# fnysalehi/Surface-Irradiance-Estimation-from-Neural-Radiance-Fields

Hardware: AMD Instinct MI355X
Metric: Mrays/s @1080p NeRF inference (Lego snapshot); PSNR vs reference (higher is better)
Workload: dtype f16; 1 GPU; Lego-shaped synthetic scene (HashGrid L8 F4 T2^19 b=2.0, density MLP 32-64-16, rgb MLP 32-64-64-16, aabb_scale 1), 1920x1080 pinhole camera fov_x 0.6911 rad, 8 orbit azimuths, 1 spp, render_mode Shade, min_transmittance 0.01; frames_in_flight=2

## Files before the change

__graft_entry__.py:

```python
import importlib
import os
import sys

ROOT = os.path.dirname(os.path.abspath(__file__))
PKG = "surface-irradiance-estimation-from-neural-radiance-fields_amd"
if ROOT not in sys.path:
    sys.path.insert(0, ROOT)


def _pkg(sub):
    return importlib.import_module(PKG + "." + sub)


def build():
    lib = _pkg("build").build()
    _pkg("build").build(legacy=True)
    _pkg("build").build_pyngp()
    _pkg("build").build_main()
    sys.path.insert(0, os.path.join(ROOT, "oracle"))
    import oracle as orc

    orc.build()
    native = _pkg("native")
    L = native.load_library()
    missing = [s for s in native.EXPORTS if not hasattr(L, s)]
    if missing:
        raise RuntimeError(f"libngp_hip.so lacks symbols: {missing}")
    print(f"built {lib}; {L.ngp_version().decode()}")


def smoke():
    import numpy as np

    sys.path.insert(0, os.path.join(ROOT, "oracle"))
    import oracle as orc

    native, synthetic, scene = _pkg("native"), _pkg("synthetic"), _pkg("scene")
    sc = synthetic.make_scene(aabb_scale=1, seed=7, log2_hashmap_size=15)
    ctx = native.Context(0)
    ctx.set_model(sc)
    w, h = 96, 54
    mat = scene.orbit_camera(45.0)
    focal = scene.focal_from_fov_x(w, 0.6911)
    img, depth = ctx.render(native.make_camera(mat, w, h, focal), native.make_opts(), want_depth=True)
    st = ctx.render_stats()
    o = orc.Oracle()
    bf, _ = o.density_grid_to_bitfield(np.asarray(sc["density_grid"], np.float16).astype(np.float32), sc["max_cascade"])
    sc["density_grid_bitfield"] = bf
    m = o.make_model(sc)
# ... 30 lines not shown
```

surface-irradiance-estimation-from-neural-radiance-fields_amd/build.py:

```python
import os
import subprocess
import sys

HERE = os.path.dirname(os.path.abspath(__file__))
CSRC = os.path.join(HERE, "csrc")
LIB = os.path.join(HERE, "libngp_hip.so")
SOURCES = ["nerf_kernels.hip", "wide_kernels.hip", "mesh_kernels.hip", "train_kernels.hip", "mc_kernels.hip", "ngp_api.cpp", "ngp_model.cpp", "ngp_snapshot.cpp", "ngp_dataset.cpp", "ngp_render.cpp", "ngp_mesh.cpp", "ngp_train.cpp", "ngp_multi.cpp", "ngp_mc.cpp"]
FLAGS = ["--offload-arch=gfx950", "-O3", "-std=c++17", "-fPIC", "-shared", "-ffp-contract=off", "-fno-slp-vectorize", "-fvisibility=hidden", "-Wall", "-Wno-unused-function"]


def hipcc():
    for c in (os.environ.get("HIPCC"), "/opt/rocm/bin/hipcc", "hipcc"):
        if c and (os.path.isabs(c) and os.path.exists(c) or not os.path.isabs(c)):
            return c
    raise RuntimeError("hipcc not found")


LIB_LEGACY = os.path.join(HERE, "libngp_hip_legacy.so")


def needs_build(lib=LIB):
    if not os.path.exists(lib):
        return True
    t = os.path.getmtime(lib)
    for f in os.listdir(CSRC):
        if os.path.getmtime(os.path.join(CSRC, f)) > t:
            return True
    inc = os.path.join(HERE, "..", "include", "ngp_hip.h")
    return os.path.getmtime(inc) > t


def build(force=False, verbose=False, legacy=False):
    lib = LIB_LEGACY if legacy else LIB
    if not force and not needs_build(lib):
        return lib
    srcs = [os.path.join(CSRC, s) for s in SOURCES if os.path.exists(os.path.join(CSRC, s))]
    tmp = "%s.%d.tmp" % (lib, os.getpid())
    cmd = [hipcc()] + FLAGS + (["-DNGP_TCNN_LEGACY_ENCODE"] if legacy else []) + os.environ.get("NGP_BUILD_DEFINES", "").split() + ["-o", tmp] + srcs + ["-lz"]
    if verbose:
        print(" ".join(cmd))
    r = subprocess.run(cmd, capture_output=True, text=True)
    if r.returncode != 0:
        sys.stderr.write(r.stdout + r.stderr)
        if os.path.exists(tmp):
            os.remove(tmp)
        raise RuntimeError("hipcc failed")
    os.replace(tmp, lib)
    return lib


def pyngp_path():
    import sysconfig

    return os.path.join(HERE, "pyngp" + sysconfig.get_config_var("EXT_SUFFIX"))


def build_pyngp(force=False, verbose=False):
    import pybind11
    import sysconfig

    out = pyngp_path()
    srcs = [os.path.join(CSRC, "pyngp.cpp"), os.path.join(CSRC, "testbed_shim.h"), os.path.join(HERE, "..", "include", "ngp_hip.h")]
    if not force and os.path.exists(out) and all(os.path.getmtime(out) >= os.path.getmtime(s) for s in srcs):
        return out
    build()
    cmd = ["g++", "-O2", "-std=c++17", "-shared", "-fPIC", "-fvisibility=hidden", "-I", sysconfig.get_paths()["include"], "-I", pybind11.get_include(),
           srcs[0], "-o", out + ".%d.tmp" % os.getpid(), "-L", HERE, "-lngp_hip", "-Wl,-rpath,$ORIGIN"]
    if verbose:
        print(" ".join(cmd))
    r = subprocess.run(cmd, capture_output=True, text=True)
    if r.returncode != 0:
# ... 41 lines not shown
```

surface-irradiance-estimation-from-neural-radiance-fields_amd/csrc/nerf_device.h:

```cpp
#pragma once

#include "ngp_kernels.h"

namespace ngp {

typedef _Float16 half_t;
typedef _Float16 half8 __attribute__((ext_vector_type(8)));
typedef float floatx4 __attribute__((ext_vector_type(4)));

struct f3 {
	float x, y, z;
};

#define NGP_DEV __device__ __forceinline__

NGP_DEV f3 mk3(float x, float y, float z) { return f3{x, y, z}; }
NGP_DEV f3 add3(f3 a, f3 b) { return mk3(a.x + b.x, a.y + b.y, a.z + b.z); }
NGP_DEV f3 sub3(f3 a, f3 b) { return mk3(a.x - b.x, a.y - b.y, a.z - b.z); }
NGP_DEV f3 mul3(f3 a, f3 b) { return mk3(a.x * b.x, a.y * b.y, a.z * b.z); }
NGP_DEV f3 div3(f3 a, f3 b) { return mk3(a.x / b.x, a.y / b.y, a.z / b.z); }
NGP_DEV f3 scale3(f3 a, float s) { return mk3(a.x * s, a.y * s, a.z * s); }
NGP_DEV f3 adds3(f3 a, float s) { return mk3(a.x + s, a.y + s, a.z + s); }
NGP_DEV float dot3(f3 a, f3 b) { return (a.x * b.x + a.y * b.y) + a.z * b.z; }
NGP_DEV f3 normalize3(f3 a) {
	float len = __builtin_sqrtf(dot3(a, a));
	return mk3(a.x / len, a.y / len, a.z / len);
}
NGP_DEV f3 m3_mulv(const float* m, f3 v) {
	f3 r = mk3(m[0] * v.x, m[1] * v.x, m[2] * v.x);
	r = add3(r, mk3(m[3] * v.y, m[4] * v.y, m[5] * v.y));
	r = add3(r, mk3(m[6] * v.z, m[7] * v.z, m[8] * v.z));
	return r;
}

NGP_DEV uint32_t laine_karras_permutation(uint32_t x, uint32_t seed) {
// ... 603 lines not shown
}
NGP_DEV float product_hi(float w, uint32_t packed) {
	float p;
	asm("v_fma_mix_f32 %0, %1, %2, 0 op_sel:[0,1,0] op_sel_hi:[0,1,0]" : "=v"(p) : "v"(w), "v"(packed));
	return p;
}
NGP_DEV void accumulate_corner(uint2 v, float w, FeatureAcc& r) {
#ifndef NGP_TCNN_LEGACY_ENCODE
	const half2_t wh = {(half_t)w, (half_t)w};
	const uint32_t wv = __builtin_bit_cast(uint32_t, wh);
	uint32_t a01 = __builtin_bit_cast(uint32_t, r.f01), a23 = __builtin_bit_cast(uint32_t, r.f23);
	asm("v_pk_fma_f16 %0, %1, %2, %0" : "+v"(a01) : "v"(wv), "v"(v.x));
	asm("v_pk_fma_f16 %0, %1, %2, %0" : "+v"(a23) : "v"(wv), "v"(v.y));
	r.f01 = __builtin_bit_cast(half2_t, a01);
	r.f23 = __builtin_bit_cast(half2_t, a23);
#else
	half2_t a, b;
	a[0] = (half_t)product_lo(w, v.x);
	a[1] = (half_t)product_hi(w, v.x);
	b[0] = (half_t)product_lo(w, v.y);
	b[1] = (half_t)product_hi(w, v.y);
	r.f01 = r.f01 + a;
	r.f23 = r.f23 + b;
#endif
}
NGP_DEV void store_features(const FeatureAcc& lo, const FeatureAcc& hi, half8& out) {
	out[0] = lo.f01[0]; out[1] = lo.f01[1]; out[2] = lo.f23[0]; out[3] = lo.f23[1];
	out[4] = hi.f01[0]; out[5] = hi.f01[1]; out[6] = hi.f23[0]; out[7] = hi.f23[1];
}

struct EncodeInFlight {
	uint2 v[16];
	float wx[2], wy[2], wz[2];
};
NGP_DEV void encode_issue(GridRsrc grid, GridRsrc xgrid, const LevelInfo* lv, int h, float x, float y, float z, EncodeInFlight& e) {
	const LevelInfo& L0 = lv[h];
	const LevelInfo& L1 = lv[h + 4];
	const CellPos p0 = level_cell(L0, x, y, z), p1 = level_cell(L1, x, y, z);
	CornerSet c0, c1;
	if (__all((int)level_in_xor_range(L0, p0) & (int)level_in_xor_range(L1, p1))) {
		level_corners_xor(L0, p0, c0);
		level_corners_xor(L1, p1, c1);
#pragma unroll
		for (int c = 0; c < 8; ++c) e.v[c] = gather8(xgrid, c0.index[c]);
#pragma unroll
		for (int c = 0; c < 8; ++c) e.v[8 + c] = gather8(xgrid, c1.index[c]);
#if defined(NGP_EXPERIMENT_EXTRA_GATHERS)
#pragma unroll
		for (int c = 0; c < NGP_EXPERIMENT_EXTRA_GATHERS; ++c) {
			const uint2 d = gather8(xgrid, c & 1 ? c1.index[c & 7] : c0.index[c & 7]);
			asm volatile("" ::"v"(d.x), "v"(d.y));
		}
#endif
	} else {
		level_corners(L0, p0, c0);
		level_corners(L1, p1, c1);
#pragma unroll
		for (int c = 0; c < 8; ++c) e.v[c] = gather8(grid, c0.index[c]);
#pragma unroll
		for (int c = 0; c < 8; ++c) e.v[8 + c] = gather8(grid, c1.index[c]);
	}
	e.wx[0] = p0.wx; e.wy[0] = p0.wy; e.wz[0] = p0.wz;
	e.wx[1] = p1.wx; e.wy[1] = p1.wy; e.wz[1] = p1.wz;
}
NGP_DEV half8 encode_finish(const EncodeInFlight& e) {
	FeatureAcc acc[2] = {{{0, 0}, {0, 0}}, {{0, 0}, {0, 0}}};
#pragma unroll
	for (int l = 0; l < 2; ++l) {
		CellPos p;
		p.gx = p.gy = p.gz = 0;
		p.wx = e.wx[l]; p.wy = e.wy[l]; p.wz = e.wz[l];
		float w[8];
		corner_weights(p, w);
#pragma unroll
		for (int c = 0; c < 8; ++c) accumulate_corner(e.v[8 * l + c], w[c], acc[l]);
	}
	half8 out;
	store_features(acc[0], acc[1], out);
	return out;
}
NGP_DEV half8 encode_level_pair(GridRsrc grid, GridRsrc xgrid, const LevelInfo* lv, int h, float x, float y, float z) {
	EncodeInFlight e;
	encode_issue(grid, xgrid, lv, h, x, y, z, e);
	return encode_finish(e);
}

NGP_DEV void sh4_quad(int h, float dx01, float dy01, float dz01, float* out4) {
	float x = dx01 * 2.0f - 1.0f, y = dy01 * 2.0f - 1.0f, z = dz01 * 2.0f - 1.0f;
	float xy = x * y, xz = x * z, yz = y * z, x2 = x * x, y2 = y * y, z2 = z * z;
	float o[16];
	o[0] = 0.28209479177387814f;
	o[1] = -0.48860251190291987f * y;
	o[2] = 0.48860251190291987f * z;
	o[3] = -0.48860251190291987f * x;
	o[4] = 1.0925484305920792f * xy;
	o[5] = -1.0925484305920792f * yz;
	o[6] = 0.94617469575755997f * z2 - 0.31539156525251999f;
	o[7] = -1.0925484305920792f * xz;
	o[8] = 0.54627421529603959f * x2 - 0.54627421529603959f * y2;
	o[9] = 0.59004358992664352f * y * (-3.0f * x2 + y2);
	o[10] = 2.8906114426405538f * xy * z;
	o[11] = 0.45704579946446572f * y * (1.0f - 5.0f * z2);
	o[12] = 0.3731763325901154f * z * (5.0f * z2 - 3.0f);
	o[13] = 0.45704579946446572f * x * (1.0f - 5.0f * z2);
	o[14] = 1.4453057213202769f * z * (x2 - y2);
	o[15] = 0.59004358992664352f * x * (-x2 + 3.0f * y2);
#pragma unroll
	for (int j = 0; j < 4; ++j) {
		float a = h == 0 ? o[j] : o[4 + j];
		float b = h == 2 ? o[8 + j] : o[12 + j];
		out4[j] = h < 2 ? a : b;
	}
}
// ... 255 lines not shown
```

surface-irradiance-estimation-from-neural-radiance-fields_amd/csrc/nerf_kernels.hip:

```cpp
#include "render_common.h"
#include "pcg32.h"

namespace ngp {

constexpr int BLOCK = 256;

struct FusedGeneric {
	static constexpr bool probe = false, unit = false, outside = true, plain = false, normals = false;
	static constexpr int prof = 0, mips = (int)NERF_CASCADES, rgb_mid = 1;
};
struct FusedUnit : FusedGeneric { static constexpr bool unit = true; static constexpr int mips = 1; };
struct FusedUnitPlain : FusedUnit { static constexpr bool plain = true; };
struct FusedC5 : FusedGeneric { static constexpr bool outside = false; static constexpr int mips = 4; };
struct FusedC5Plain : FusedC5 { static constexpr bool plain = true; };
struct FusedMid0 : FusedGeneric { static constexpr int rgb_mid = 0; };
struct FusedMid2 : FusedGeneric { static constexpr int rgb_mid = 2; };
struct FusedLinRgb : FusedGeneric { static constexpr int rgb_mid = -1; };
struct FusedLin : FusedGeneric { static constexpr int rgb_mid = -2; };
struct FusedNormals : FusedGeneric { static constexpr bool normals = true; };
struct FusedProf : FusedGeneric { static constexpr int prof = 1; };
struct FusedUnitPlainProf : FusedUnitPlain { static constexpr int prof = 1; };
struct FusedUnitPlainProf2 : FusedUnitPlain { static constexpr int prof = 2; };
struct FusedProbe : FusedGeneric { static constexpr bool probe = true; };

template <class V>
NGP_DEV void fused_body(const ModelParams& M, const CameraParams& C, const FrameParams& F, const ProbeParams& P) {
	constexpr bool PROBE = V::probe, UNIT = V::unit, OUTSIDE = V::outside, PLAIN = V::plain, NORMALS = V::normals;
	constexpr int PROF = V::prof, MIPS = V::mips, RGB_MID = V::rgb_mid;
	const uint32_t max_cascade = UNIT ? 0u : M.max_cascade;
	const float cone_angle = UNIT ? 0.0f : M.cone_angle;
	const Stepping stepping = make_stepping(cone_angle);
	__shared__ uint4 s_w[n_frags_for(RGB_MID) * 64];
	__shared__ LevelInfo s_lv[N_LEVELS];
	__shared__ uint32_t s_coarse[MIPS * COARSE_WORDS_PER_MIP];
	__shared__ uint32_t s_coarse16[(UNIT ? 1 : (int)NERF_CASCADES) * 16];
	__shared__ uint2 s_sh[BLOCK * 4];
	constexpr int SLOTS = 64;
	__shared__ float4 s_samp[BLOCK / 64 * SLOTS];
	__shared__ uint2 s_res[BLOCK / 64 * SLOTS];
	__shared__ float4 s_nrm[NORMALS ? BLOCK / 64 * SLOTS : 1];
	__shared__ uint32_t s_xstate, s_xcount, s_active;
	constexpr uint32_t XRAYS = 16;
	__shared__ float s_xray[XRAYS * 16];
	if (threadIdx.x == 0) {
		s_xstate = 0u;
		s_xcount = 0u;
		s_active = BLOCK / 64;
	}
	unsigned long long t_entry = 0, rt_entry = 0;
	if (PROF) { t_entry = stamp(); rt_entry = realtime(); }
	for (int i = threadIdx.x; i < n_frags_for(RGB_MID) * 64; i += BLOCK) s_w[i] = M.wfrags[i];
	if (threadIdx.x < N_LEVELS) s_lv[threadIdx.x] = M.levels[threadIdx.x];
	for (uint32_t i = threadIdx.x; i < (max_cascade + 1 < (uint32_t)MIPS ? max_cascade + 1 : (uint32_t)MIPS) * COARSE_WORDS_PER_MIP; i += BLOCK) s_coarse[i] = M.coarse[i];
	if (threadIdx.x < (UNIT ? 1 : (int)NERF_CASCADES) * 16) s_coarse16[threadIdx.x] = M.coarse[NERF_CASCADES * COARSE_WORDS_PER_MIP + threadIdx.x];
	__syncthreads();

	const int lane = threadIdx.x & 63;
	const int c = lane & 15;
	if (lane == 0 && (threadIdx.x >> 6) == 0) atomicMax(&F.results[4], ~realtime());
	const GridRsrc t_grid = make_grid_rsrc(M.grid, M.grid_bytes), t_xgrid = make_grid_rsrc(M.xgrid, M.xgrid_bytes);
	const float* cam_last = (!PLAIN && C.moving) ? C.m1 : C.m;
	const f3 cam_fwd = mk3(cam_last[6], cam_last[7], cam_last[8]);
	const f3 bg_linear = (PROBE || !F.direct) ? mk3(0.f, 0.f, 0.f)
	                     : F.color_space == 1 ? mk3(F.background[0], F.background[1], F.background[2])
	                                          : mk3(srgb_to_linear(F.background[0]), srgb_to_linear(F.background[1]), srgb_to_linear(F.background[2]));
	const float4 empty_pixel = (!PROBE && F.direct) ? tonemap_pixel(F, bg_linear, 0.f, 0.f, 0.f, 0.f) : make_float4(0.f, 0.f, 0.f, 0.f);
	const f3 cam_pos = mk3(cam_last[9], cam_last[10], cam_last[11]);
	const f3 amin = mk3(M.aabb_min[0], M.aabb_min[1], M.aabb_min[2]);
	const f3 adiag = mk3(M.aabb_diag[0], M.aabb_diag[1], M.aabb_diag[2]);

	RayState ray;
	ray.alive = false;
	ray.o = ray.d = mk3(0.f, 0.f, 0.f);
	ray.t = 0.f;
	ray.idx = 0;
	ray.out = 0;
	f3 idir = mk3(0.f, 0.f, 0.f);
	Accum acc = {0.f, 0.f, 0.f, 0.f, 0.f, 0.f};
	uint32_t step = 1;
	uint32_t skip_i = 1;
	float t_max = 0.f;
	bool counted = false;
	uint32_t n_pend = 0, sl_lo = 0, sl_hi = 0;
	bool left_box = false;
	uint32_t n_slots = 0;
	const int wave_base = threadIdx.x & ~63;
	OccBlock occ_cache;
	occ_cache.key = 0xffffffffu;
	occ_cache.bits = make_uint2(0u, 0u);
	bool finished = false;
	bool idle = false;
	const uint32_t my_wave = threadIdx.x >> 6;

	bool exhausted = false;
	uint32_t qsel = (uint32_t)__builtin_amdgcn_s_getreg(20 | (0 << 6) | (3 << 11)) & 7u;
	int stall = 0;
	uint32_t n_alive_init = 0, n_hit = 0, n_samples = 0;
	unsigned long long p_skip[3] = {0, 0, 0};
	unsigned long long pt[4] = {0, 0, 0, 0}, p_iters = 0, p_passes = 0, p_rounds = 0, p_lane_steps = 0, t0 = 0, t1 = 0;

	unsigned long long rt_start = 0;
	if (PROF && F.prof) {
		rt_start = realtime();
		if (lane == 0) atomicMax(&F.prof[8], ~rt_start);
	}
	int tr_slot = -1;
	uint32_t tr_it = 0, tr_info0 = 0, tr_info1 = 0, tr_march = 0;
	uint32_t tr_net[5] = {0, 0, 0, 0, 0};
	unsigned long long tr_t[5] = {0, 0, 0, 0, 0};
	auto trace_emit = [&](int upto) {
		if (!PROF || tr_slot < 0) return;
		if (tr_it < F.trace_cap_iters && lane == 0) {
			uint32_t* r = F.trace + 16 + F.trace_cap_waves * 16u + ((size_t)tr_slot * F.trace_cap_iters + tr_it) * 16u;
			r[0] = (uint32_t)tr_t[0];
			for (int k = 1; k < 5; ++k) r[k] = (uint32_t)(tr_t[k <= upto ? k : upto] - tr_t[0]);
			r[5] = tr_info0;
			r[6] = tr_info1;
			r[7] = tr_march;
			for (int k = 0; k < 5; ++k) r[8 + k] = upto >= 3 ? tr_net[k] : 0u;
		}
		++tr_it;
	};
	for (;;) {
		if (PROF) { t0 = stamp(); tr_t[0] = t0; tr_info0 = tr_info1 = tr_march = 0; for (int k = 0; k < 5; ++k) tr_net[k] = 0; }
		unsigned long long dead_mask = __ballot(!ray.alive);
		int n_dead = __popcll(dead_mask);
		if ((exhausted || n_dead >= F.tune[0]) && __any(finished)) {
			bool hit = false;
			if (finished) {
				hit = shade_ray<PROBE, PLAIN, NORMALS>(F, P, bg_linear, ray.out, acc, step - 1u, ray.d);
				finished = false;
			}
			n_hit += (uint32_t)__popcll(__ballot(hit));
			if (PROF) tr_info1 |= 4u << 24;
		}
		if (!exhausted && n_dead >= (F.tune[0] > 16 ? F.tune[0] : 16)) {
			const uint32_t want = (uint32_t)n_dead >> 4, n_strips = F.n_local_tiles * 4u;
			uint32_t first = 0, limit = n_strips;
			if (!PROBE && F.xqueue) {
				for (int tries = 0; tries < 8; ++tries) {
					const uint32_t lo = (uint32_t)(((unsigned long long)n_strips * qsel) >> 3), hi = (uint32_t)(((unsigned long long)n_strips * (qsel + 1u)) >> 3);
					uint32_t off = 0;
					if (lane == 0) off = atomicAdd(F.xqueue + qsel, want);
					off = __builtin_amdgcn_readfirstlane(off);
					first = lo + off;
					limit = hi;
					if (off < hi - lo) break;
					first = limit = n_strips;
					qsel = (qsel + 1u) & 7u;
				}
			} else {
				if (lane == 0) first = atomicAdd(F.queue, want);
				first = __builtin_amdgcn_readfirstlane(first);
			}
			if (first >= limit) {
				exhausted = true;
			} else {
// ... 282 lines not shown
		const int hq = lane >> 4;
		auto sample_of = [&](int p, float& sx, float& sy, float& sz, Sh4& shq) {
			const float4 a = s_samp[wave_base + 16 * p + c];
			const uint32_t owner = s_res[wave_base + 16 * p + c].x;
			sx = a.x; sy = a.y; sz = a.z;
			union { uint2 u; half_t h[4]; } cv;
			cv.u = s_sh[(wave_base + (int)owner) * 4 + hq];
#pragma unroll
			for (int j = 0; j < 4; ++j) shq.v[j] = cv.h[j];
		};
		auto deliver = [&](int p, const MlpOut& mo) {
			union { half_t h[4]; uint2 u; } o;
			o.h[0] = mo.rgb[0]; o.h[1] = mo.rgb[1]; o.h[2] = mo.rgb[2]; o.h[3] = mo.sigma;
			if (lane < 16) s_res[wave_base + 16 * p + lane] = o.u;
		};
		int p = 0;
		if (NORMALS) {
			for (; p < n_pass; ++p) {
				float ax, ay, az;
				Sh4 sha;
				sample_of(p, ax, ay, az, sha);
				EncodeInFlight e;
				encode_issue(t_grid, t_xgrid, s_lv, hq, ax, ay, az, e);
				const half8 enc = encode_finish(e);
				DensityGrad dg = density_gradient_pass(s_w, M.wfrags, lane, e, enc, s_lv[hq].scale, s_lv[hq + 4].scale, M.density_linear != 0);
#pragma unroll
				for (int k = 0; k < 3; ++k) {
					dg.g[k] += __shfl_xor(dg.g[k], 16, 64);
					dg.g[k] += __shfl_xor(dg.g[k], 32, 64);
				}
				if (lane < 16) s_nrm[wave_base + 16 * p + lane] = make_float4(dg.g[0] * (1.0f / 128.0f), dg.g[1] * (1.0f / 128.0f), dg.g[2] * (1.0f / 128.0f), (float)dg.sigma);
			}
		}
		unsigned long long u0 = 0, u1 = 0;
		auto lap = [&](int k, bool drain_gathers) {
			if (drain_gathers) asm volatile("s_waitcnt vmcnt(0)" ::: "memory");
			u1 = stamp();
			tr_net[k] += (uint32_t)(u1 - u0);
			u0 = u1;
		};
		if (PROF >= 2) u0 = stamp();
		for (; p + 1 < n_pass; p += 2) {
			float ax, ay, az, bx, by, bz;
			Sh4 sha, shb;
			sample_of(p, ax, ay, az, sha);
			sample_of(p + 1, bx, by, bz, shb);
			EncodeInFlight ea, eb;
			encode_issue(t_grid, t_xgrid, s_lv, hq, ax, ay, az, ea);
			encode_issue(t_grid, t_xgrid, s_lv, hq, bx, by, bz, eb);
			if (PROF >= 2) { lap(0, false); lap(1, true); }
			half8 enca = encode_finish(ea);
			half8 encb = encode_finish(eb);
			if (PROF >= 2) lap(2, false);
			MlpOut moa = mlp_pass<RGB_MID>(s_w, lane, enca, sha);
			MlpOut mob = mlp_pass<RGB_MID>(s_w, lane, encb, shb);
			if (PROF >= 2) lap(3, false);
			deliver(p, moa);
			deliver(p + 1, mob);
			if (PROF >= 2) lap(4, false);
		}
		if (p < n_pass) {
			float ax, ay, az;
			Sh4 sha;
			sample_of(p, ax, ay, az, sha);
			EncodeInFlight e1;
			encode_issue(t_grid, t_xgrid, s_lv, hq, ax, ay, az, e1);
			if (PROF >= 2) { lap(0, false); lap(1, true); }
			half8 enc = encode_finish(e1);
			if (PROF >= 2) lap(2, false);
			MlpOut mo = mlp_pass<RGB_MID>(s_w, lane, enc, sha);
			if (PROF >= 2) lap(3, false);
			deliver(p, mo);
			if (PROF >= 2) lap(4, false);
		}

		if (PROF) { t1 = stamp(); pt[2] += t1 - t0; t0 = t1; p_passes += (unsigned long long)n_pass; tr_t[3] = t1; tr_info0 |= (n_slots << 8) | ((uint32_t)n_pass << 16); }
		for (uint32_t k = 0;; ++k) {
			const bool have = k < n_pend && ray.alive;
			if (!__any(have)) break;
			if (have) {
				const uint32_t slot = ((k < 4u ? sl_lo >> (8u * k) : sl_hi >> (8u * (k - 4u))) & 0xffu);
				const float4 a = s_samp[wave_base + slot];
				union { uint2 u; half_t h[4]; } o;
				o.u = s_res[wave_base + slot];
				float gx = 0.f, gy = 0.f, gz = 0.f;
				if (NORMALS) {
					const float4 g = s_nrm[wave_base + slot];
					gx = g.x; gy = g.y; gz = g.z;
					o.h[3] = (half_t)g.w;
				}
				const f3 pos = add3(amin, mul3(mk3(a.x, a.y, a.z), adiag));
				const float sdepth = PROBE ? dot3(ray.d, sub3(pos, ray.o))
				                          : dot3(cam_fwd, sub3(pos, cam_pos));
				float T = 1.0f - acc.a;
				float dt = unwarp_dt(a.w);
				float alpha = 1.0f - fast_exp(-network_to_density((float)o.h[3], M.density_act) * dt);
				float weight = alpha * T;
				float cr = network_to_rgb((float)o.h[0], M.rgb_act), cg = network_to_rgb((float)o.h[1], M.rgb_act), cb = network_to_rgb((float)o.h[2], M.rgb_act);
				if (!PROBE && F.render_mode > 1) {
					if (NORMALS) {
						const float dd = network_to_density_derivative((float)o.h[3], M.density_act);
						const f3 nrm = normalize3(mk3(-dd * gx, -dd * gy, -dd * gz));
// ... 31 lines not shown
		}
		left_box = false;
		n_pend = 0;
		sl_lo = sl_hi = 0;
		n_slots = 0;
		if (PROF) { t1 = stamp(); pt[3] += t1 - t0; tr_t[4] = t1; trace_emit(4); }
	}
	if (PROF) {
		for (int k = 0; k < 3; ++k)
			for (int off = 32; off > 0; off >>= 1) p_skip[k] += __shfl_down(p_skip[k], off, 64);
	}
	if (PROF && tr_slot >= 0 && lane == 0) {
		uint32_t* hd = F.trace + 16 + (size_t)tr_slot * 16u;
		const unsigned long long rt_end = realtime(), t_end = stamp();
		hd[4] = tr_it;
		hd[7] = (uint32_t)rt_end; hd[8] = (uint32_t)(rt_end >> 32);
		hd[12] = (uint32_t)t_end;
		hd[13] = n_samples;
	}
	if (PROF && lane == 0 && F.prof) {
		for (int k = 0; k < 3; ++k) atomicAdd(&F.prof[12 + k], p_skip[k]);
		for (int k = 0; k < 4; ++k) atomicAdd(&F.prof[k], pt[k]);
		atomicAdd(&F.prof[4], p_iters);
		atomicAdd(&F.prof[5], p_passes);
		atomicAdd(&F.prof[6], p_rounds);
		atomicAdd(&F.prof[7], p_lane_steps);
		unsigned long long t_end = realtime(), t_first = ~F.prof[8];
		atomicMax(&F.prof[9], t_end);
		unsigned long long bucket = (t_end - t_first) / 10000ull;
		if (bucket > 47ull) bucket = 47ull;
		atomicAdd(&F.prof[16 + bucket], 1ull);
	}

	finish_launch(F, lane, n_alive_init, n_hit, n_samples);
}

#define NGP_FUSED_KERNEL(NAME, WAVES, V) \
	__global__ __launch_bounds__(BLOCK, WAVES) void NAME(const ModelParams M, const CameraParams C, const FrameParams F) { \
		ProbeParams P{}; \
		fused_body<V>(M, C, F, P); \
	}
NGP_FUSED_KERNEL(render_nerf_fused, 2, FusedGeneric)
NGP_FUSED_KERNEL(render_nerf_fused_unit, 3, FusedUnit)
NGP_FUSED_KERNEL(render_nerf_fused_unit_plain, 3, FusedUnitPlain)
NGP_FUSED_KERNEL(render_nerf_fused_c5_plain, 3, FusedC5Plain)
NGP_FUSED_KERNEL(render_nerf_fused_c5, 3, FusedC5)
NGP_FUSED_KERNEL(render_nerf_fused_mid0, 2, FusedMid0)
NGP_FUSED_KERNEL(render_nerf_fused_mid2, 2, FusedMid2)
NGP_FUSED_KERNEL(render_nerf_fused_lin_rgb, 2, FusedLinRgb)
NGP_FUSED_KERNEL(render_nerf_fused_lin, 2, FusedLin)
NGP_FUSED_KERNEL(render_nerf_fused_normals, 2, FusedNormals)
NGP_FUSED_KERNEL(render_nerf_fused_prof, 2, FusedProf)
NGP_FUSED_KERNEL(render_nerf_fused_unit_plain_prof, 3, FusedUnitPlainProf)
NGP_FUSED_KERNEL(render_nerf_fused_unit_plain_prof2, 3, FusedUnitPlainProf2)

__global__ __launch_bounds__(BLOCK, 2) void trace_probe_fused(const ModelParams M, const FrameParams F, const ProbeParams P) {
	CameraParams C{};
	fused_body<FusedProbe>(M, C, F, P);
}

__global__ void probe_reduce_kernel(const ProbeParams P, float4* __restrict__ envmap) {
	uint32_t texel = blockIdx.x * blockDim.x + threadIdx.x;
	const uint32_t per_probe = P.n_theta * P.n_phi, n_probes = P.mode == 3 ? P.grid_x * P.grid_y : 1u;
	if (texel >= per_probe * n_probes) return;
	if (P.mode == 3) {
		envmap[texel] = P.ray_rgba[texel];
// ... 360 lines not shown
}

template <typename K>
static int resident_blocks_per_cu(K kernel) {
	int n = 0;
	if (hipOccupancyMaxActiveBlocksPerMultiprocessor(&n, kernel, BLOCK, 0) != hipSuccess || n < 1) n = 1;
	return n;
}
static int grid_blocks(const FrameParams& F, int resident) {
	const int waves = BLOCK / 64, needed = (int)((F.n_local_tiles + waves - 1) / waves);
	return resident > needed ? (needed > 0 ? needed : 1) : resident;
}
static FrameParams with_grid(const FrameParams& F, int n_blocks) {
	FrameParams G = F;
	G.n_waves = (uint32_t)n_blocks * (BLOCK / 64);
	return G;
}
static int head_kind(const ModelParams& M) { return M.rgb_mid < 0 ? (M.density_linear ? -2 : -1) : M.rgb_mid; }

enum RenderKernel { RK_GENERIC, RK_UNIT, RK_UNIT_PLAIN, RK_C5, RK_C5_PLAIN, RK_PROF, RK_UNIT_PLAIN_PROF, RK_UNIT_PLAIN_PROF2,
                    RK_MID0, RK_MID2, RK_LIN_RGB, RK_LIN, RK_NORMALS, RK_COUNT, RK_WIDE = RK_COUNT };
static RenderKernel select_render_kernel(const ModelParams& M, const CameraParams& C, const FrameParams& F) {
	if (M.wide.width) return RK_WIDE;
	if (F.render_mode == 7) return RK_NORMALS;
	switch (head_kind(M)) {
	case -2: return RK_LIN;
	case -1: return RK_LIN_RGB;
	case 0: return RK_MID0;
	case 2: return RK_MID2;
	}
	const bool unit = M.max_cascade == 0 && M.cone_angle <= 1e-5f;
	const bool c5 = !unit && M.max_cascade < 5 && !F.outside_possible;
	const bool plain = C.lens_mode == 0 && C.aperture_size == 0.0f && !C.moving && !F.envmap;
	if (F.prof) return unit && plain ? (F.prof_level >= 2 ? RK_UNIT_PLAIN_PROF2 : RK_UNIT_PLAIN_PROF) : RK_PROF;
	if (unit) return plain ? RK_UNIT_PLAIN : RK_UNIT;
	if (c5) return plain ? RK_C5_PLAIN : RK_C5;
	return RK_GENERIC;
}
static const struct { void (*kernel)(ModelParams, CameraParams, FrameParams); bool clamped; } RENDER_KERNELS[RK_COUNT] = {
	{render_nerf_fused, true}, {render_nerf_fused_unit, true}, {render_nerf_fused_unit_plain, true}, {render_nerf_fused_c5, true},
	{render_nerf_fused_c5_plain, true}, {render_nerf_fused_prof, true}, {render_nerf_fused_unit_plain_prof, true},
	{render_nerf_fused_unit_plain_prof2, true}, {render_nerf_fused_mid0, false}, {render_nerf_fused_mid2, false},
	{render_nerf_fused_lin_rgb, false}, {render_nerf_fused_lin, false}, {render_nerf_fused_normals, false}};
void launch_render_nerf_wide(const ModelParams& M, const CameraParams& C, const FrameParams& F, int n_cus, hipStream_t stream);
void launch_trace_probe_wide(const ModelParams& M, const FrameParams& F, const ProbeParams& P, int n_cus, hipStream_t stream);
void launch_render_nerf(const ModelParams& M, const CameraParams& C, const FrameParams& F, int n_cus, hipStream_t stream) {
	const RenderKernel k = select_render_kernel(M, C, F);
	if (k == RK_WIDE) return launch_render_nerf_wide(M, C, F, n_cus, stream);
	static const struct PerCu { int v[RK_COUNT]; } resident = []() {
		PerCu r;
		for (int i = 0; i < RK_COUNT; ++i) r.v[i] = resident_blocks_per_cu(RENDER_KERNELS[i].kernel);
		return r;
	}();
	int per_cu = resident.v[k];
	if (RENDER_KERNELS[k].clamped) {
		static const int shard_per_cu = []() { const char* e = getenv("NGP_SHARD_BLOCKS_PER_CU"); int v = e ? atoi(e) : 2; return v >= 1 && v <= 8 ? v : 2; }();
		if (F.shard_count > 1 && per_cu > shard_per_cu) per_cu = shard_per_cu;
		if (F.shard_count <= 1 && F.n_local_tiles <= 6144u && per_cu > 2) per_cu = 2;
		if (const char* e = getenv("NGP_BLOCKS_PER_CU")) { int v = atoi(e); if (v > 0 && v < per_cu) per_cu = v; }
	}
	const int n_blocks = grid_blocks(F, n_cus * per_cu);
	const FrameParams G = with_grid(F, n_blocks);
	hipLaunchKernelGGL(RENDER_KERNELS[k].kernel, dim3(n_blocks), dim3(BLOCK), 0, stream, M, C, G);
}
void launch_trace_probe(const ModelParams& M, const FrameParams& F, const ProbeParams& P, int n_cus, hipStream_t stream) {
	if (M.wide.width) return launch_trace_probe_wide(M, F, P, n_cus, stream);
	static const int per_cu = resident_blocks_per_cu(trace_probe_fused);
// ... 111 lines not shown
```

surface-irradiance-estimation-from-neural-radiance-fields_amd/csrc/ngp_render.cpp:

```cpp
#include "ngp_host.h"

#include <map>
#include <mutex>

#include <algorithm>
#include <cmath>
#include <cstdio>
#include <cstring>

using namespace ngp;

namespace {

uint32_t reverse_bits32(uint32_t x) {
	x = ((x & 0xaaaaaaaau) >> 1) | ((x & 0x55555555u) << 1);
	x = ((x & 0xccccccccu) >> 2) | ((x & 0x33333333u) << 2);
	x = ((x & 0xf0f0f0f0u) >> 4) | ((x & 0x0f0f0f0fu) << 4);
	x = ((x & 0xff00ff00u) >> 8) | ((x & 0x00ff00ffu) << 8);
	return (x >> 16) | (x << 16);
}
uint32_t lk_perm(uint32_t x, uint32_t seed) {
	x += seed;
	x ^= x * 0x6c50b47cu;
	x ^= x * 0xb82f1e52u;
// ... 41 lines not shown
	const uint32_t shard_count = shard_count_of(opts);
	F.frame_buffer = ctx->d_frame.get();
	F.depth_buffer = d_depth_out ? d_depth_out : ctx->d_depth.get();
	ctx->bind_slot(F, slot);
	if (shard_count > 1) F.xqueue = nullptr;
	F.tiles_x = (uint32_t)(cam.width + 7) / 8;
	F.tiles_y = (uint32_t)(cam.height + 7) / 8;
	F.shard_index = opts.shard_index;
	F.shard_count = shard_count;
	F.n_local_tiles = tile_share(cam.width, cam.height, opts.shard_index, shard_count);
	F.min_transmittance = opts.min_transmittance;
	F.linear_colors = ctx->desc.linear_colors;
	F.packed = opts.packed_output ? 1 : 0;
	F.prof = nullptr;
	memcpy(F.tune, ctx->tune, sizeof(F.tune));
	if (getenv("NGP_PROFILE_SECTIONS")) {
		if (!ctx->d_prof) ctx->d_prof.reset(128);
		NGP_HIP_CHECK(hipMemsetAsync(ctx->d_prof.get(), 0, 1024, stream));
		F.prof = ctx->d_prof.get();
		F.prof_level = atoi(getenv("NGP_PROFILE_SECTIONS"));
		if (const char* e = getenv("NGP_PROFILE_TRACE")) {
			const int stride = atoi(e);
			if (stride > 0) {
				const size_t words = 16 + (size_t)ngp_ctx::TRACE_WAVES * 16 + (size_t)ngp_ctx::TRACE_WAVES * ngp_ctx::TRACE_ITERS * 16;
				if (!ctx->d_trace) ctx->d_trace.reset(words);
				NGP_HIP_CHECK(hipMemsetAsync(ctx->d_trace.get(), 0, words * sizeof(uint32_t), stream));
				F.trace = ctx->d_trace.get();
				F.trace_stride = (uint32_t)stride;
				F.trace_cap_waves = ngp_ctx::TRACE_WAVES;
				F.trace_cap_iters = ngp_ctx::TRACE_ITERS;
			}
		}
	}
	const bool geometry = opts.testbed_mode == NGP_MODE_GEOMETRY;
	const bool have_meshes = geometry && !ctx->meshes.empty();
	if (have_meshes && cam.has_matrix1 && memcmp(cam.matrix, cam.matrix1, sizeof(cam.matrix)) != 0) throw std::runtime_error("a moving camera (matrix1 / rolling shutter) renders NeRF mode");
	F.depth_test = geometry ? 1 : 0;
	if (have_meshes) {
		for (int i = 0; i < 3; ++i) { M.raabb_min[i] = ctx->mesh_scene.scene_min[i]; M.raabb_max[i] = ctx->mesh_scene.scene_max[i]; }
		const float ident[9] = {1, 0, 0, 0, 1, 0, 0, 0, 1};
		memcpy(M.r2l, ident, sizeof(ident));
		M.r2l_identity = 1u;
	}

	F.direct = (spp == 1 && !have_meshes && !geometry && (shard_count == 1 || opts.packed_output)) ? 1 : 0;
	F.to_srgb = opts.to_srgb;
	F.render_mode = opts.render_mode == NGP_RENDER_SHADE_GRID_ENVMAP ? NGP_RENDER_SHADE_ENVMAP : opts.render_mode;
	F.color_space = opts.color_space;
	if (opts.color_space != 0 && opts.color_space != 1) throw std::runtime_error("color_space: 0 (Linear) or 1 (SRGB)");
	F.depth_scale = opts.depth_scale != 0.f ? opts.depth_scale : 1.0f / 0.33f;
	memcpy(F.background, opts.background, sizeof(F.background));
	F.exposure_scale = powf(2.0f, opts.exposure);
	if (ctx->d_bg_envmap) {
		if (geometry) throw std::runtime_error("an environment map applies to NeRF mode (in the reference the Geometry-mode NeRF pass would paint it over the meshes, src/testbed_geometry_training.cu:1993-1995): clear it with ngp_set_envmap(ctx, 0, 0, NULL)");
		F.envmap = ctx->d_bg_envmap.get();
		F.env_w = ctx->bg_env_w;
		F.env_h = ctx->bg_env_h;
	}
	{
		const float h = 0.5f * (float)(1u << M.max_cascade);
		bool inside = M.r2l_identity != 0;
		for (int i = 0; i < 3; ++i) inside = inside && M.raabb_min[i] >= 0.5f - h && M.raabb_max[i] <= 0.5f + h;
		F.outside_possible = inside ? 0 : 1;
	}
}

// ... 235 lines not shown
	});
}

static void read_history_slot(ngp_ctx* ctx, uint64_t call, ngp_render_stats* out) {
	const int slot = (int)(call % ngp_ctx::HISTORY);
	unsigned long long c[4];
	NGP_HIP_CHECK(hipMemcpy(c, ctx->d_sync.get() + ngp_ctx::SLOT_BYTES * (size_t)slot + 32, sizeof(c), hipMemcpyDeviceToHost));
	out->kernel_device_ms = (float)((double)c[3] * 1e-5);
	out->n_rays = ctx->hist_n_rays[slot];
	out->n_rays_alive_after_init = c[0];
	out->n_rays_hit = c[1];
	out->n_samples = c[2];
	NGP_HIP_CHECK(hipEventElapsedTime(&out->kernel_ms, ctx->ev_kern0[slot], ctx->ev_kern1[slot]));
	NGP_HIP_CHECK(hipEventElapsedTime(&out->frame_ms, ctx->ev_frame0[slot], ctx->ev_frame1[slot]));
}

int ngp_get_render_stats(ngp_ctx* ctx, ngp_render_stats* out) {
	return guarded(ctx, [&] {
		if (!out) throw std::runtime_error("null argument");
		if (!ctx->n_calls) throw std::runtime_error("nothing rendered yet");
		NGP_HIP_CHECK(hipStreamSynchronize(ctx->last_stream));
		read_history_slot(ctx, ctx->n_calls - 1, out);
		if (ctx->last_was_multi) {
			for (ngp_ctx* p : ctx->peers) {
				ngp_render_stats s{};
				DeviceGuard g(p->device);
				if (ngp_get_render_stats(p, &s) != 0) throw std::runtime_error(p->error);
				out->n_rays += s.n_rays; out->n_rays_alive_after_init += s.n_rays_alive_after_init; out->n_rays_hit += s.n_rays_hit; out->n_samples += s.n_samples;
				out->kernel_ms = std::max(out->kernel_ms, s.kernel_ms);
				out->frame_ms = std::max(out->frame_ms, s.frame_ms);
				out->kernel_device_ms = std::max(out->kernel_device_ms, s.kernel_device_ms);
			}
		}
		if (ctx->d_prof && getenv("NGP_PROFILE_SECTIONS")) {
			unsigned long long p[128];
			NGP_HIP_CHECK(hipMemcpy(p, ctx->d_prof.get(), sizeof(p), hipMemcpyDeviceToHost));
			{
				const double us = 0.01, t_first = (double)(~p[8]);
				fprintf(stderr, "[ngp timeline] kernel %.1f us | queue empty seen first at %.1f us, last at %.1f us | wave exits per 0.1 ms:", ((double)p[9] - t_first) * us,
				        ((double)(~p[10]) - t_first) * us, ((double)p[11] - t_first) * us);
				for (int b = 0; b < 48; ++b) fprintf(stderr, " %llu", p[16 + b]);
				fprintf(stderr, "\n[ngp skips] lane-steps that left an empty cell %llu, an empty 4^3 block %llu, an empty 16^3 block %llu\n", p[12], p[13], p[14]);
			}
			double tot = (double)(p[0] + p[1] + p[2] + p[3]);
			fprintf(stderr, "[ngp profile] refill %.1f%% march %.1f%% network %.1f%% composite %.1f%% | wave-iterations %llu passes %llu | cycles/iter %.0f cycles/pass(network) %.0f | skip rounds %llu lane-steps %llu (%.1f lanes/round) cycles/round %.0f\n",
			        100.0 * p[0] / tot, 100.0 * p[1] / tot, 100.0 * p[2] / tot, 100.0 * p[3] / tot, p[4], p[5], tot / (double)p[4], (double)p[2] / (double)p[5], p[6], p[7], (double)p[7] / (double)p[6], (double)p[1] / (double)p[6]);
			if (ctx->M.wide.width && p[5])
				fprintf(stderr, "[ngp wide profile] per network round: hidden layers %.0f (-) %.0f output layers %.0f | march loop %.0f decision %.0f rows+prefetch %.0f encode %.0f composite %.0f | rounds %llu network rounds %llu\n",
				        (double)p[64] / p[5], (double)p[65] / p[5], (double)p[71] / p[5], (double)p[66] / p[5], (double)p[67] / p[5], (double)p[68] / p[5], (double)p[69] / p[5], (double)p[70] / p[5], p[4], p[5]);
		}
	});
}

int ngp_get_profile_trace(ngp_ctx* ctx, uint32_t* out, uint64_t n_words, uint32_t* cap_waves, uint32_t* cap_iters) {
	return guarded(ctx, [&] {
		if (!ctx->d_trace) throw std::runtime_error("no wave trace: set NGP_PROFILE_SECTIONS=1|2 and NGP_PROFILE_TRACE=<stride> before rendering");
		const size_t words = 16 + (size_t)ngp_ctx::TRACE_WAVES * 16 + (size_t)ngp_ctx::TRACE_WAVES * ngp_ctx::TRACE_ITERS * 16;
		if (cap_waves) *cap_waves = ngp_ctx::TRACE_WAVES;
		if (cap_iters) *cap_iters = ngp_ctx::TRACE_ITERS;
		if (!out) return;
		NGP_HIP_CHECK(hipDeviceSynchronize());
		NGP_HIP_CHECK(hipMemcpy(out, ctx->d_trace.get(), std::min<size_t>(words, (size_t)n_words) * sizeof(uint32_t), hipMemcpyDeviceToHost));
	});
}

int ngp_set_schedule(ngp_ctx* ctx, const int32_t* knobs, int n) {
// ... 37 lines not shown
```

Baseline: 1062 Mrays/s.

## Cache coarse-level hash-grid corner features per wave in shared memory

Adds a small set-associative per-wave cache in LDS, holding the 8 corner feature vectors of the coarse level in each level pair, keyed by cell coordinates. In the unit-cascade fused kernel, a sample that hits the cache reads its corners from shared memory instead of issuing 8 global gathers, and misses refill the line after the encode. The aim is to cut redundant gathers for neighbouring samples that fall in the same coarse cell. The cost is extra LDS, which may lower occupancy, plus tag checks and LDS traffic, and races between lanes writing the same set are resolved by re-checking the tag. Also adds nocache and statistics build variants.

```diff
diff --git a/__graft_entry__.py b/__graft_entry__.py
--- a/__graft_entry__.py
+++ b/__graft_entry__.py
@@ -15,6 +15,7 @@
 def build():
     lib = _pkg("build").build()
     _pkg("build").build(legacy=True)
+    _pkg("build").build(nocache=True)
     _pkg("build").build_pyngp()
     _pkg("build").build_main()
     sys.path.insert(0, os.path.join(ROOT, "oracle"))
diff --git a/surface-irradiance-estimation-from-neural-radiance-fields_amd/build.py b/surface-irradiance-estimation-from-neural-radiance-fields_amd/build.py
--- a/surface-irradiance-estimation-from-neural-radiance-fields_amd/build.py
+++ b/surface-irradiance-estimation-from-neural-radiance-fields_amd/build.py
@@ -17,6 +17,8 @@
 
 
 LIB_LEGACY = os.path.join(HERE, "libngp_hip_legacy.so")
+LIB_CELLSTATS = os.path.join(HERE, "libngp_hip_cellstats.so")
+LIB_NOCACHE = os.path.join(HERE, "libngp_hip_nocache.so")
 
 
 def needs_build(lib=LIB):
@@ -30,13 +32,15 @@
     return os.path.getmtime(inc) > t
 
 
-def build(force=False, verbose=False, legacy=False):
-    lib = LIB_LEGACY if legacy else LIB
+def build(force=False, verbose=False, legacy=False, nocache=False, cellstats=False):
+    if legacy + nocache + cellstats > 1:
+        raise ValueError("one variant at a time")
+    lib = LIB_LEGACY if legacy else LIB_NOCACHE if nocache else LIB_CELLSTATS if cellstats else LIB
     if not force and not needs_build(lib):
         return lib
     srcs = [os.path.join(CSRC, s) for s in SOURCES if os.path.exists(os.path.join(CSRC, s))]
     tmp = "%s.%d.tmp" % (lib, os.getpid())
-    cmd = [hipcc()] + FLAGS + (["-DNGP_TCNN_LEGACY_ENCODE"] if legacy else []) + os.environ.get("NGP_BUILD_DEFINES", "").split() + ["-o", tmp] + srcs + ["-lz"]
+    cmd = [hipcc()] + FLAGS + (["-DNGP_TCNN_LEGACY_ENCODE"] if legacy else []) + (["-DNGP_NO_CELL_CACHE"] if nocache else []) + (["-DNGP_EXPERIMENT_CELL_CACHE_STATS"] if cellstats else []) + os.environ.get("NGP_BUILD_DEFINES", "").split() + ["-o", tmp] + srcs + ["-lz"]
     if verbose:
         print(" ".join(cmd))
     r = subprocess.run(cmd, capture_output=True, text=True)
diff --git a/surface-irradiance-estimation-from-neural-radiance-fields_amd/csrc/cell_cache.h b/surface-irradiance-estimation-from-neural-radiance-fields_amd/csrc/cell_cache.h
--- /dev/null
+++ b/surface-irradiance-estimation-from-neural-radiance-fields_amd/csrc/cell_cache.h
@@ -0,0 +1,24 @@
+#pragma once
+#include <stdint.h>
+
+#if defined(__HIPCC__) || defined(__CUDACC__)
+#define NGP_CELL_FN __host__ __device__ __forceinline__
+#else
+#define NGP_CELL_FN inline
+#endif
+
+namespace ngp {
+
+constexpr int CELL_CACHE_LEVELS = 4;
+constexpr uint32_t CELL_COORD_MAX = 255u;
+constexpr uint32_t CELL_TAG_NONE = 0xFFFFFFFFu;
+
+NGP_CELL_FN bool cell_cacheable(uint32_t gx, uint32_t gy, uint32_t gz) { return ((gx | gy | gz) >> 8) == 0u; }
+NGP_CELL_FN uint32_t cell_tag(uint32_t gx, uint32_t gy, uint32_t gz) { return gx | (gy << 8) | (gz << 16); }
+NGP_CELL_FN uint32_t cell_set(uint32_t tag, uint32_t n_sets) {
+	const uint32_t lo = (tag & 1u) | ((tag >> 7) & 2u) | ((tag >> 14) & 4u);
+	const uint32_t hi = ((tag >> 1) ^ (tag >> 9) ^ (tag >> 17)) & 1u;
+	return (lo | (hi << 3)) & (n_sets - 1u);
+}
+
+}
diff --git a/surface-irradiance-estimation-from-neural-radiance-fields_amd/csrc/nerf_device.h b/surface-irradiance-estimation-from-neural-radiance-fields_amd/csrc/nerf_device.h
--- a/surface-irradiance-estimation-from-neural-radiance-fields_amd/csrc/nerf_device.h
+++ b/surface-irradiance-estimation-from-neural-radiance-fields_amd/csrc/nerf_device.h
@@ -1,6 +1,7 @@
 #pragma once
 
 #include "ngp_kernels.h"
+#include "cell_cache.h"
 
 namespace ngp {
 
@@ -670,6 +671,7 @@
 struct EncodeInFlight {
 	uint2 v[16];
 	float wx[2], wy[2], wz[2];
+	uint32_t cell;
 };
 NGP_DEV void encode_issue(GridRsrc grid, GridRsrc xgrid, const LevelInfo* lv, int h, float x, float y, float z, EncodeInFlight& e) {
 	const LevelInfo& L0 = lv[h];
@@ -717,6 +719,63 @@
 	store_features(acc[0], acc[1], out);
 	return out;
 }
+constexpr int CELL_CACHE_SETS = 8;
+struct CellCache {
+	uint4 line[CELL_CACHE_LEVELS][CELL_CACHE_SETS][4];
+	uint32_t tag[CELL_CACHE_LEVELS][CELL_CACHE_SETS];
+};
+NGP_DEV void cell_cache_clear(CellCache* caches, int n_waves, int thread, int n_threads) {
+	for (int i = thread; i < n_waves * CELL_CACHE_LEVELS * CELL_CACHE_SETS; i += n_threads)
+		caches[i / (CELL_CACHE_LEVELS * CELL_CACHE_SETS)].tag[i / CELL_CACHE_SETS % CELL_CACHE_LEVELS][i % CELL_CACHE_SETS] = CELL_TAG_NONE;
+}
+NGP_DEV void encode_issue_cached(GridRsrc grid, GridRsrc xgrid, const LevelInfo* lv, int h, float x, float y, float z, EncodeInFlight& e, CellCache& cc) {
+	const LevelInfo& L0 = lv[h];
+	const LevelInfo& L1 = lv[h + 4];
+	const CellPos p0 = level_cell(L0, x, y, z), p1 = level_cell(L1, x, y, z);
+	CornerSet c0, c1;
+	e.cell = CELL_TAG_NONE;
+	if (__all((int)level_in_xor_range(L0, p0) & (int)level_in_xor_range(L1, p1))) {
+		level_corners_xor(L1, p1, c1);
+#pragma unroll
+		for (int c = 0; c < 8; ++c) e.v[8 + c] = gather8(xgrid, c1.index[c]);
+		const bool cacheable = cell_cacheable(p0.gx, p0.gy, p0.gz);
+		const uint32_t tag = cell_tag(p0.gx, p0.gy, p0.gz), set = cell_set(tag, CELL_CACHE_SETS);
+		const bool hit = __hip_atomic_load(&cc.tag[h][set], __ATOMIC_RELAXED, __HIP_MEMORY_SCOPE_WAVEFRONT) == tag && cacheable;
+#pragma unroll
+		for (int q = 0; q < 4; ++q) {
+			const uint4 d = cc.line[h][set][q];
+			e.v[2 * q] = make_uint2(d.x, d.y);
+			e.v[2 * q + 1] = make_uint2(d.z, d.w);
+		}
+		if (!hit) {
+			level_corners_xor(L0, p0, c0);
+#pragma unroll
+			for (int c = 0; c < 8; ++c) e.v[c] = gather8(xgrid, c0.index[c]);
+			if (cacheable) e.cell = tag;
+		}
+	} else {
+		level_corners(L0, p0, c0);
+		level_corners(L1, p1, c1);
+#pragma unroll
+		for (int c = 0; c < 8; ++c) e.v[c] = gather8(grid, c0.index[c]);
+#pragma unroll
+		for (int c = 0; c < 8; ++c) e.v[8 + c] = gather8(grid, c1.index[c]);
+	}
+	e.wx[0] = p0.wx; e.wy[0] = p0.wy; e.wz[0] = p0.wz;
+	e.wx[1] = p1.wx; e.wy[1] = p1.wy; e.wz[1] = p1.wz;
+}
+NGP_DEV void cell_cache_fill(CellCache& cc, int h, const EncodeInFlight& e) {
+	if (e.cell != CELL_TAG_NONE) {
+		const uint32_t set = cell_set(e.cell, CELL_CACHE_SETS);
+		__hip_atomic_store(&cc.tag[h][set], e.cell, __ATOMIC_RELAXED, __HIP_MEMORY_SCOPE_WAVEFRONT);
+		asm volatile("" ::: "memory");
+		if (__hip_atomic_load(&cc.tag[h][set], __ATOMIC_RELAXED, __HIP_MEMORY_SCOPE_WAVEFRONT) == e.cell) {
+#pragma unroll
+			for (int q = 0; q < 4; ++q) cc.line[h][set][q] = make_uint4(e.v[2 * q].x, e.v[2 * q].y, e.v[2 * q + 1].x, e.v[2 * q + 1].y);
+		}
+	}
+}
+
 NGP_DEV half8 encode_level_pair(GridRsrc grid, GridRsrc xgrid, const LevelInfo* lv, int h, float x, float y, float z) {
 	EncodeInFlight e;
 	encode_issue(grid, xgrid, lv, h, x, y, z, e);
diff --git a/surface-irradiance-estimation-from-neural-radiance-fields_amd/csrc/nerf_kernels.hip b/surface-irradiance-estimation-from-neural-radiance-fields_amd/csrc/nerf_kernels.hip
--- a/surface-irradiance-estimation-from-neural-radiance-fields_amd/csrc/nerf_kernels.hip
+++ b/surface-irradiance-estimation-from-neural-radiance-fields_amd/csrc/nerf_kernels.hip
@@ -5,11 +5,16 @@
 
 constexpr int BLOCK = 256;
 
+#if defined(NGP_NO_CELL_CACHE) || defined(NGP_EXPERIMENT_CELL_CACHE_STATS)
+constexpr bool CELL_CACHE_BUILT = false;
+#else
+constexpr bool CELL_CACHE_BUILT = true;
+#endif
 struct FusedGeneric {
-	static constexpr bool probe = false, unit = false, outside = true, plain = false, normals = false;
+	static constexpr bool probe = false, unit = false, outside = true, plain = false, normals = false, cell_cache = false;
 	static constexpr int prof = 0, mips = (int)NERF_CASCADES, rgb_mid = 1;
 };
-struct FusedUnit : FusedGeneric { static constexpr bool unit = true; static constexpr int mips = 1; };
+struct FusedUnit : FusedGeneric { static constexpr bool unit = true, cell_cache = CELL_CACHE_BUILT; static constexpr int mips = 1; };
 struct FusedUnitPlain : FusedUnit { static constexpr bool plain = true; };
 struct FusedC5 : FusedGeneric { static constexpr bool outside = false; static constexpr int mips = 4; };
 struct FusedC5Plain : FusedC5 { static constexpr bool plain = true; };
@@ -25,7 +30,7 @@
 
 template <class V>
 NGP_DEV void fused_body(const ModelParams& M, const CameraParams& C, const FrameParams& F, const ProbeParams& P) {
-	constexpr bool PROBE = V::probe, UNIT = V::unit, OUTSIDE = V::outside, PLAIN = V::plain, NORMALS = V::normals;
+	constexpr bool PROBE = V::probe, UNIT = V::unit, OUTSIDE = V::outside, PLAIN = V::plain, NORMALS = V::normals, CELL_CACHE = V::cell_cache;
 	constexpr int PROF = V::prof, MIPS = V::mips, RGB_MID = V::rgb_mid;
 	const uint32_t max_cascade = UNIT ? 0u : M.max_cascade;
 	const float cone_angle = UNIT ? 0.0f : M.cone_angle;
@@ -39,6 +44,12 @@
 	__shared__ float4 s_samp[BLOCK / 64 * SLOTS];
 	__shared__ uint2 s_res[BLOCK / 64 * SLOTS];
 	__shared__ float4 s_nrm[NORMALS ? BLOCK / 64 * SLOTS : 1];
+	__shared__ CellCache s_cells[CELL_CACHE ? BLOCK / 64 : 1];
+#ifdef NGP_EXPERIMENT_CELL_CACHE_STATS
+	__shared__ uint32_t s_cst[BLOCK / 64][CELL_CACHE_LEVELS][4 + 8 + 16];
+	for (int i = threadIdx.x; i < BLOCK / 64 * CELL_CACHE_LEVELS * 28; i += BLOCK) (&s_cst[0][0][0])[i] = CELL_TAG_NONE;
+	unsigned long long cst_n = 0, cst_hit[3] = {0, 0, 0};
+#endif
 	__shared__ uint32_t s_xstate, s_xcount, s_active;
 	constexpr uint32_t XRAYS = 16;
 	__shared__ float s_xray[XRAYS * 16];
@@ -53,6 +64,7 @@
 	if (threadIdx.x < N_LEVELS) s_lv[threadIdx.x] = M.levels[threadIdx.x];
 	for (uint32_t i = threadIdx.x; i < (max_cascade + 1 < (uint32_t)MIPS ? max_cascade + 1 : (uint32_t)MIPS) * COARSE_WORDS_PER_MIP; i += BLOCK) s_coarse[i] = M.coarse[i];
 	if (threadIdx.x < (UNIT ? 1 : (int)NERF_CASCADES) * 16) s_coarse16[threadIdx.x] = M.coarse[NERF_CASCADES * COARSE_WORDS_PER_MIP + threadIdx.x];
+	if (CELL_CACHE) cell_cache_clear(s_cells, BLOCK / 64, threadIdx.x, BLOCK);
 	__syncthreads();
 
 	const int lane = threadIdx.x & 63;
@@ -106,7 +118,7 @@
 	}
 	int tr_slot = -1;
 	uint32_t tr_it = 0, tr_info0 = 0, tr_info1 = 0, tr_march = 0;
-	uint32_t tr_net[5] = {0, 0, 0, 0, 0};
+	uint32_t tr_net[7] = {0, 0, 0, 0, 0, 0, 0};
 	unsigned long long tr_t[5] = {0, 0, 0, 0, 0};
 	auto trace_emit = [&](int upto) {
 		if (!PROF || tr_slot < 0) return;
@@ -117,12 +129,12 @@
 			r[5] = tr_info0;
 			r[6] = tr_info1;
 			r[7] = tr_march;
-			for (int k = 0; k < 5; ++k) r[8 + k] = upto >= 3 ? tr_net[k] : 0u;
+			for (int k = 0; k < 7; ++k) r[8 + k] = upto >= 3 ? tr_net[k] : 0u;
 		}
 		++tr_it;
 	};
 	for (;;) {
-		if (PROF) { t0 = stamp(); tr_t[0] = t0; tr_info0 = tr_info1 = tr_march = 0; for (int k = 0; k < 5; ++k) tr_net[k] = 0; }
+		if (PROF) { t0 = stamp(); tr_t[0] = t0; tr_info0 = tr_info1 = tr_march = 0; for (int k = 0; k < 7; ++k) tr_net[k] = 0; }
 		unsigned long long dead_mask = __ballot(!ray.alive);
 		int n_dead = __popcll(dead_mask);
 		if ((exhausted || n_dead >= F.tune[0]) && __any(finished)) {
@@ -471,9 +483,36 @@
 				if (lane < 16) s_nrm[wave_base + 16 * p + lane] = make_float4(dg.g[0] * (1.0f / 128.0f), dg.g[1] * (1.0f / 128.0f), dg.g[2] * (1.0f / 128.0f), (float)dg.sigma);
 			}
 		}
+		auto issue = [&](float sx, float sy, float sz, EncodeInFlight& e) {
+			if constexpr (CELL_CACHE) encode_issue_cached(t_grid, t_xgrid, s_lv, hq, sx, sy, sz, e, s_cells[my_wave]);
+			else encode_issue(t_grid, t_xgrid, s_lv, hq, sx, sy, sz, e);
+#ifdef NGP_EXPERIMENT_CELL_CACHE_STATS
+			const CellPos p = level_cell(s_lv[hq], sx, sy, sz);
+			e.cell = CELL_TAG_NONE;
+			if (level_in_xor_range(s_lv[hq], p) && cell_cacheable(p.gx, p.gy, p.gz)) {
+				const uint32_t tag = cell_tag(p.gx, p.gy, p.gz);
+				e.cell = tag;
+				++cst_n;
+				for (int k = 0; k < 3; ++k) {
+					const bool hit = s_cst[my_wave][hq][(4 << k) - 4 + cell_set(tag, 4u << k)] == tag;
+					cst_hit[k] += hit ? 1u : 0u;
+					e.cell |= hit ? 0u : 1u << (24 + k);
+				}
+			}
+#endif
+		};
+		auto keep = [&](const EncodeInFlight& e) {
+			if constexpr (CELL_CACHE) cell_cache_fill(s_cells[my_wave], hq, e);
+#ifdef NGP_EXPERIMENT_CELL_CACHE_STATS
+			if (e.cell != CELL_TAG_NONE)
+				for (int k = 0; k < 3; ++k)
+					if (e.cell >> (24 + k) & 1u) s_cst[my_wave][hq][(4 << k) - 4 + cell_set(e.cell & 0xFFFFFFu, 4u << k)] = e.cell & 0xFFFFFFu;
+#endif
+		};
 		unsigned long long u0 = 0, u1 = 0;
 		auto lap = [&](int k, bool drain_gathers) {
 			if (drain_gathers) asm volatile("s_waitcnt vmcnt(0)" ::: "memory");
+			else if (k == 5) asm volatile("s_waitcnt lgkmcnt(0)" ::: "memory");
 			u1 = stamp();
 			tr_net[k] += (uint32_t)(u1 - u0);
 			u0 = u1;
@@ -485,12 +524,15 @@
 			sample_of(p, ax, ay, az, sha);
 			sample_of(p + 1, bx, by, bz, shb);
 			EncodeInFlight ea, eb;
-			encode_issue(t_grid, t_xgrid, s_lv, hq, ax, ay, az, ea);
-			encode_issue(t_grid, t_xgrid, s_lv, hq, bx, by, bz, eb);
-			if (PROF >= 2) { lap(0, false); lap(1, true); }
+			issue(ax, ay, az, ea);
+			issue(bx, by, bz, eb);
+			if (PROF >= 2) { lap(0, false); if (CELL_CACHE) lap(5, false); lap(1, true); }
 			half8 enca = encode_finish(ea);
 			half8 encb = encode_finish(eb);
 			if (PROF >= 2) lap(2, false);
+			keep(ea);
+			keep(eb);
+			if (PROF >= 2 && CELL_CACHE) lap(6, false);
 			MlpOut moa = mlp_pass<RGB_MID>(s_w, lane, enca, sha);
 			MlpOut mob = mlp_pass<RGB_MID>(s_w, lane, encb, shb);
 			if (PROF >= 2) lap(3, false);
@@ -503,10 +545,12 @@
 			Sh4 sha;
 			sample_of(p, ax, ay, az, sha);
 			EncodeInFlight e1;
-			encode_issue(t_grid, t_xgrid, s_lv, hq, ax, ay, az, e1);
-			if (PROF >= 2) { lap(0, false); lap(1, true); }
+			issue(ax, ay, az, e1);
+			if (PROF >= 2) { lap(0, false); if (CELL_CACHE) lap(5, false); lap(1, true); }
 			half8 enc = encode_finish(e1);
 			if (PROF >= 2) lap(2, false);
+			keep(e1);
+			if (PROF >= 2 && CELL_CACHE) lap(6, false);
 			MlpOut mo = mlp_pass<RGB_MID>(s_w, lane, enc, sha);
 			if (PROF >= 2) lap(3, false);
 			deliver(p, mo);
@@ -604,6 +648,18 @@
 		atomicAdd(&F.prof[16 + bucket], 1ull);
 	}
 
+#ifdef NGP_EXPERIMENT_CELL_CACHE_STATS
+	if (F.prof) {
+		for (int off = 8; off > 0; off >>= 1) {
+			cst_n += __shfl_xor(cst_n, off, 64);
+			for (int k = 0; k < 3; ++k) cst_hit[k] += __shfl_xor(cst_hit[k], off, 64);
+		}
+		if (c == 0) {
+			atomicAdd(&F.prof[64 + 4 * (lane >> 4)], cst_n);
+			for (int k = 0; k < 3; ++k) atomicAdd(&F.prof[64 + 4 * (lane >> 4) + 1 + k], cst_hit[k]);
+		}
+	}
+#endif
 	finish_launch(F, lane, n_alive_init, n_hit, n_samples);
 }
 
@@ -1030,7 +1086,11 @@
 	const bool unit = M.max_cascade == 0 && M.cone_angle <= 1e-5f;
 	const bool c5 = !unit && M.max_cascade < 5 && !F.outside_possible;
 	const bool plain = C.lens_mode == 0 && C.aperture_size == 0.0f && !C.moving && !F.envmap;
-	if (F.prof) return unit && plain ? (F.prof_level >= 2 ? RK_UNIT_PLAIN_PROF2 : RK_UNIT_PLAIN_PROF) : RK_PROF;
+	bool stamped = F.prof != nullptr;
+#ifdef NGP_EXPERIMENT_CELL_CACHE_STATS
+	stamped = stamped && F.prof_level > 0;
+#endif
+	if (stamped) return unit && plain ? (F.prof_level >= 2 ? RK_UNIT_PLAIN_PROF2 : RK_UNIT_PLAIN_PROF) : RK_PROF;
 	if (unit) return plain ? RK_UNIT_PLAIN : RK_UNIT;
 	if (c5) return plain ? RK_C5_PLAIN : RK_C5;
 	return RK_GENERIC;
diff --git a/surface-irradiance-estimation-from-neural-radiance-fields_amd/csrc/ngp_render.cpp b/surface-irradiance-estimation-from-neural-radiance-fields_amd/csrc/ngp_render.cpp
--- a/surface-irradiance-estimation-from-neural-radiance-fields_amd/csrc/ngp_render.cpp
+++ b/surface-irradiance-estimation-from-neural-radiance-fields_amd/csrc/ngp_render.cpp
@@ -97,6 +97,15 @@
 			}
 		}
 	}
+#ifdef NGP_EXPERIMENT_CELL_CACHE_STATS
+	if (!F.prof) {
+		if (!ctx->d_prof) {
+			ctx->d_prof.reset(128);
+			NGP_HIP_CHECK(hipMemsetAsync(ctx->d_prof.get(), 0, 1024, stream));
+		}
+		F.prof = ctx->d_prof.get();
+	}
+#endif
 	const bool geometry = opts.testbed_mode == NGP_MODE_GEOMETRY;
 	const bool have_meshes = geometry && !ctx->meshes.empty();
 	if (have_meshes && cam.has_matrix1 && memcmp(cam.matrix, cam.matrix1, sizeof(cam.matrix)) != 0) throw std::runtime_error("a moving camera (matrix1 / rolling shutter) renders NeRF mode");
@@ -398,6 +407,14 @@
 				out->kernel_device_ms = std::max(out->kernel_device_ms, s.kernel_device_ms);
 			}
 		}
+#ifdef NGP_EXPERIMENT_CELL_CACHE_STATS
+		if (ctx->d_prof) {
+			unsigned long long p[128];
+			NGP_HIP_CHECK(hipMemcpy(p, ctx->d_prof.get(), sizeof(p), hipMemcpyDeviceToHost));
+			for (int l = 0; l < 4; ++l)
+				fprintf(stderr, "[ngp cell cache] level %d lookups %llu hits with 4 / 8 / 16 sets %llu %llu %llu\n", l, p[64 + 4 * l], p[65 + 4 * l], p[66 + 4 * l], p[67 + 4 * l]);
+		}
+#endif
 		if (ctx->d_prof && getenv("NGP_PROFILE_SECTIONS")) {
 			unsigned long long p[128];
 			NGP_HIP_CHECK(hipMemcpy(p, ctx->d_prof.get(), sizeof(p), hipMemcpyDeviceToHost));
```

Measured after the change: 1097 Mrays/s, median of 6. +3.3%, better.
